# dan-lee-gh/monte-carlo-gp

Hardware: AMD Instinct MI355X
Metric: race-simulations/sec (20 drivers, 60 laps) (higher is better)
Workload: dtype f64

## Files before the change

monte_carlo_gp_amd/csrc/race_isa.hip.h:

```cpp
#ifndef MCGP_RACE_ISA_H
#define MCGP_RACE_ISA_H
#include <hip/hip_runtime.h>

namespace mcgp {

__device__ __forceinline__ void minmax_f64(double a, double b, double &lo, double &hi)
{
    asm("v_min_f64 %0, %1, %2" : "=v"(lo) : "v"(a), "v"(b));
    asm("v_max_f64 %0, %1, %2" : "=v"(hi) : "v"(a), "v"(b));
}

__device__ __forceinline__ double max_f64(double a, double b)
{
    double r;
    asm("v_max_f64 %0, %1, %2" : "=v"(r) : "v"(a), "v"(b));
    return r;
}

__device__ __forceinline__ double max_abs_f64(double a, double b)
{
    double r;
    asm("v_max_f64 %0, |%1|, %2" : "=v"(r) : "v"(a), "v"(b));
    return r;
}
// ... 627 lines not shown
__device__ __forceinline__ void lds_ld_u32x4(uint32_t addr, uint32_t &a, uint32_t &b, uint32_t &c, uint32_t &d)
{
    typedef uint32_t v4u __attribute__((ext_vector_type(4)));
    const v4u v = *reinterpret_cast<const MCGP_LDS v4u *>(addr);
    a = v.x; b = v.y; c = v.z; d = v.w;
}
__device__ __forceinline__ void lds_ld_f64_u32x2(uint32_t addr, double &d, uint32_t &u0, uint32_t &u1)
{
    typedef uint32_t v4u __attribute__((ext_vector_type(4)));
    const v4u v = *reinterpret_cast<const MCGP_LDS v4u *>(addr);
    d = __hiloint2double((int)v.y, (int)v.x);
    u0 = v.z;
    u1 = v.w;
}

__device__ __forceinline__ uint32_t cvt_u32_f64_sat(double x)
{
    uint32_t r;
    asm("v_cvt_u32_f64 %0, %1" : "=v"(r) : "v"(x));
    return r;
}
__device__ __forceinline__ double ceil_f64(double x) { return __builtin_ceil(x); }
__device__ __forceinline__ uint32_t min_u32(uint32_t a, uint32_t b) { return a < b ? a : b; }
__device__ __forceinline__ void sched_fence() { __builtin_amdgcn_sched_barrier(0); }
__device__ __forceinline__ void wave_sync()
{
    __builtin_amdgcn_fence(__ATOMIC_RELEASE, "wavefront");
    __builtin_amdgcn_wave_barrier();
    __builtin_amdgcn_fence(__ATOMIC_ACQUIRE, "wavefront");
}
// ... 49 lines not shown
```

monte_carlo_gp_amd/csrc/race_kernel_reg.hip.h:

```cpp
#pragma once
#include "race_common.hip.h"
#include "race_isa.hip.h"
#include "sort_networks.h"

#include <utility>

#ifndef MCGP_STAT
#define MCGP_STAT(what, value)
#endif
#ifndef MCGP_TRACE_PASS
#define MCGP_TRACE_PASS(sim, lap, pass, n_cand)
#endif
#ifndef MCGP_COOPERATIVE_EVENTS
#define MCGP_COOPERATIVE_EVENTS 1
#endif
#ifndef MCGP_GRID_EXACT
#define MCGP_GRID_EXACT 0
#endif
#ifndef MCGP_WIDE_EXACT
#define MCGP_WIDE_EXACT 0
#endif
#ifndef MCGP_WIDE_TIE_SHIFT
#define MCGP_WIDE_TIE_SHIFT 0
#endif

namespace mcgp {

constexpr uint32_t k3UsedMask = 7u;
constexpr uint32_t k3Drs = 1u << 3;
constexpr int k3IdShift = 4;
constexpr uint32_t k3IdMask = 31u << k3IdShift;
constexpr uint32_t k3Dnf = 1u << 9;
constexpr uint32_t k3SlotMask = k3IdMask | k3Dnf;
constexpr int k3CompShift = 10;
constexpr uint32_t k3CompMask = 7u << k3CompShift;
constexpr uint32_t k3Dirty = 1u << 13;
constexpr int k3AgeShift = 16;
constexpr uint32_t k3AgeMask = 0x7FFu << k3AgeShift;
constexpr int k3GposShift = 27;
__host__ __device__ constexpr uint32_t pk_driver16(uint32_t p) { return p & k3IdMask; }
__host__ __device__ constexpr uint32_t pk_slot16(uint32_t p) { return p & k3SlotMask; }
__host__ __device__ constexpr uint32_t pk_comp512(uint32_t p) { return (p & k3CompMask) >> (k3CompShift - 9); }
__host__ __device__ constexpr uint32_t pk_comp16(uint32_t p) { return (p >> (k3CompShift - 4)) & 0x70u; }
constexpr double kAgeFieldUnit = 1.0 / 65536.0;

constexpr size_t kLdsPerCu = 160 * 1024;
__host__ __device__ constexpr size_t align16(size_t x) { return (x + 15) / 16 * 16; }
constexpr int kWordRows = 8;
__host__ __device__ constexpr size_t per_thread_lds_bytes_reg(int n) { return (size_t)kWordRows * 4 + (size_t)n * 8; }
constexpr int kNumCompounds = 5;
__host__ __device__ constexpr size_t shared_lds_bytes_reg(int n)
{
    return (size_t)kNormalRows * 16 + (size_t)n * 16 + (size_t)(kMaxCars + n) * 16 +
           (size_t)((kNumCompounds - 1) * kMaxCars + n) * 16 + kCompStride * 16 + 64 + 128 + align16((size_t)n * n * 4) +
           align16((size_t)n * n * 8);
}
__host__ __device__ constexpr int reg_min_waves(int n) { return n <= 6 ? (n == 4 ? 4 : 6) : n <= 11 ? 4 : n <= 22 ? 3 : 2; }
__host__ __device__ constexpr bool reg_commit_by_selects(int n) { return n == 6 || (n >= 8 && n <= 10) || n == 24 || n == 25; }
__host__ __device__ constexpr bool reg_step_by_selects(int n) { return n == 3 || n == 11 || n == 12 || n == 25 || n == 26 || n == 29; }
__host__ __device__ constexpr bool reg_update_by_selects(int n)
{
    return n == 1 || n == 6 || (n >= 9 && n <= 11) || n == 22 || n == 28 || n == 29;
}
__host__ __device__ constexpr bool reg_threshold_by_selects(int n) { return n == 6 || n == 7 || (n >= 23 && n <= 25) || n >= 27; }
constexpr int kMaxBlockWaves = 16;
constexpr size_t kLdsReserve = 256;
__host__ __device__ constexpr int block_shape_rank(int w) { return (w % 4 == 0 ? 0 : 100) + (w <= 8 ? 2 * (8 - w) : w - 8); }
__host__ __device__ constexpr int reg_block_waves(int n)
{
    const int cap = 4 * reg_min_waves(n);
// ... 23 lines not shown
    return rows > kWideLdsRowsMax ? kWideLdsRowsMax : rows;
}
__host__ __device__ constexpr size_t wide_lds_bytes(int n, int waves)
{
    return wide_fixed_lds_bytes(n, waves) + (size_t)wide_lds_rows(n, waves) * kNorm53LdsStride;
}
__host__ __device__ constexpr size_t wide_chain_bytes(int n, int total_laps)
{
    return total_laps >= 2 ? (size_t)(total_laps - 1) * (size_t)((n + 3) & ~3) * 8 : 0;
}
__host__ __device__ constexpr size_t wide_launch_lds_bytes(int n, int waves, int total_laps)
{
    const size_t base = wide_lds_bytes(n, waves), chain = wide_chain_bytes(n, total_laps);
    return base + chain + kLdsReserve <= kLdsPerCu ? base + chain : base;
}
template <int N, int WAVES = reg_block_waves(N), bool WIDE = false>
struct RegGeo {
    static constexpr int kWaves = WAVES;
    static constexpr bool kWide = WIDE;
    static constexpr int B = 64 * kWaves;
    static constexpr uint32_t oDrvA = 0;
    static constexpr uint32_t oDrvB = oDrvA + N * 16;
    static constexpr uint32_t oIc = oDrvB + (kMaxCars + N) * 16;
    static constexpr uint32_t oComp = oIc + ((kNumCompounds - 1) * kMaxCars + N) * 16;
    static constexpr uint32_t oDrs = oComp + kCompStride * 16;
    static constexpr uint32_t oPit = oDrs + 16;
    static constexpr uint32_t oDrsB = oDrs + 32;
    static constexpr uint32_t oLut = oDrsB + 32;
    static constexpr uint32_t oNorm = oLut + 128;
    static constexpr uint32_t oHist = oNorm + (WIDE ? 0 : kNormalRows * 16);
    static_assert(WIDE || oNorm >= kNormalRowBias * 16, "the inverse-normal rows are addressed through a base 48 rows before the table");
    static constexpr uint32_t oGrid = oHist + (uint32_t)align16((size_t)N * N * 4);
    static constexpr uint32_t oW = oGrid + (uint32_t)align16((size_t)N * N * 8);
    static constexpr uint32_t oLast = oW + (uint32_t)kWordRows * B * 4;
    static constexpr uint32_t oNorm53 = oLast + (uint32_t)N * B * 8;
    static constexpr int kNorm53Rows = WIDE ? wide_lds_rows(N, WAVES) : 0;
    static constexpr int kNorm53First = kNormal53Rows - kNorm53Rows;
    static constexpr uint32_t kBytes = oNorm53 + (uint32_t)kNorm53Rows * (uint32_t)kNorm53LdsStride;
    static constexpr uint32_t oChain = kBytes;
    static constexpr uint32_t kChainStride = (uint32_t)((N + 3) & ~3) * 8u;
    __host__ __device__ static constexpr bool chain_fits(int total_laps)
    {
        return WIDE && total_laps >= 2 && kBytes + wide_chain_bytes(N, total_laps) + kLdsReserve <= kLdsPerCu;
    }
    static_assert(oW == shared_lds_bytes_reg(N) - (WIDE ? (size_t)kNormalRows * 16 : 0) && oLast % 8 == 0, "LDS map");
    static_assert(oW % 16 == 0 && oNorm53 % 16 == 0, "the event handler parks fields with 16-byte LDS accesses (ds_write_b128 / ds_read_b128); table rows are read 16 bytes at a time");
    static_assert(kBytes == (WIDE ? wide_lds_bytes(N, WAVES) : per_thread_lds_bytes_reg(N) * B + shared_lds_bytes_reg(N)), "LDS map");
    static_assert(kBytes + kLdsReserve <= kLdsPerCu, "block does not fit LDS");
// ... 1 lines not shown
};
constexpr int kWideMinLdsRows = 14 * 16;
__host__ __device__ constexpr int wide_block_waves(int n)
{
    if (n <= 22) {
        for (int w = 12; w > 8; --w)
            if (wide_fixed_lds_bytes(n, w) + kLdsReserve <= kLdsPerCu && wide_lds_rows(n, w) >= kWideMinLdsRows) return w;
    }
    int w = 8;
    while (w > 1 && wide_fixed_lds_bytes(n, w) + kLdsReserve > kLdsPerCu) --w;
    return w;
}
__host__ __device__ constexpr int wide_min_waves(int n) { return wide_block_waves(n) > 8 ? 3 : 2; }
template <int N>
using WideGeo = RegGeo<N, wide_block_waves(N), true>;

template <int N>
struct SortNetwork {
    int a[N * 8];
    int b[N * 8];
    int step[N * 8];
    int n;
    int ga[N * 8];
    int gn[N * 8];
    int n_groups;
    constexpr SortNetwork() : a{}, b{}, step{}, n(0), ga{}, gn{}, n_groups(0)
    {
        const SortNetworkTable *table = nullptr;
        for (const SortNetworkTable &t : kSortNetworks)
            if (t.n == N) table = &t;
// ... 188 lines not shown
}

template <int N>
__device__ __forceinline__ bool resort_after_overtakes(double (&cum)[N], uint32_t (&pk)[N])
{
    bubble_forward<N, 0>(cum, pk);
    bubble_backward<N, N - 2>(cum, pk);
    const bool strict = strictly_increasing<N>(cum);
    MCGP_STAT(14, !strict);
    if (__builtin_expect(!strict, 0)) {
        if (!in_order<N>(cum, pk)) transposition_sort<N>(cum, pk);
    }
    return strict;
}

template <int N, bool DISTINCT = false>
__device__ __forceinline__ void update_positions_reg(const double (&cum)[N], uint32_t (&pk)[N],
                                                     bool drs_allowed, double dirty_thr)
{
    bool first = true;
    double leader = 0.0, prev = 0.0;
#pragma unroll
    for (int i = 0; i < N; ++i) {
        const uint32_t p = pk[i];
        const bool act = !(p & k3Dnf);
        const double t = cum[i];
        leader = (act && first) ? t : leader;
        const double tbl = t - leader;
        const bool dirty = (DISTINCT ? !first : tbl > 0) && tbl < dirty_thr;
        const bool drs = !first && drs_allowed && (t - prev) < 1.0;
        pk[i] = (p & ~(k3Drs | k3Dirty)) | (dirty ? k3Dirty : 0u) | (drs ? k3Drs : 0u);
        prev = act ? t : prev;
        first = first && !act;
    }
}

__host__ __device__ constexpr int pit_regime(int remaining_laps)
{
    return remaining_laps > 30 ? 0 : remaining_laps > 20 ? 1 : remaining_laps > 15 ? 2 : 3;
}
__device__ __forceinline__ uint32_t pit_rule_word(int track, int regime, uint32_t used, uint32_t pop_sh, uint32_t pop_mh)
{
    const int remaining_laps = regime == 0 ? 31 : regime == 1 ? 21 : regime == 2 ? 16 : 0;
    uint32_t newc = stint_compound(track, remaining_laps);
    if (track == 0 && __popc(used) == 1 && ((used >> newc) & 1u)) {
        const uint32_t avail = 7u & ~used;
        const uint32_t popped = avail == 5u ? pop_sh : avail == 6u ? pop_mh : 0u;
        if (remaining_laps > 20) newc = (avail & 2u) ? 1u : popped;
        else newc = (avail & 1u) ? 0u : popped;
    }
    return (newc << k3CompShift) | ((used | (1u << newc)) & k3UsedMask);
}

constexpr double kRegTimeFloor = 8.0;
__host__ __device__ inline double reg_time_floor(const KParams &kp)
{
    const double z_max = kp.wide ? 8.5 : 6.5;
    double floor_ = __builtin_inf();
    double cdelta_min = __builtin_inf();
    for (int c = 0; c < 5; ++c) cdelta_min = kp.comp_delta[c] < cdelta_min ? kp.comp_delta[c] : cdelta_min;
    for (int d = 0; d < kp.n; ++d) {
        double eff_min = 0.0;
        for (int c = 0; c < 5; ++c) {
            const double e = kp.comp_deg[c] * kp.factor[d];
            eff_min = e < eff_min ? e : eff_min;
        }
// ... 42 lines not shown
            }
        }
    } else {
        float4 *t_norm = reinterpret_cast<float4 *>(smem + G::oNorm);
        for (uint32_t i = tid; i < (uint32_t)kNormalRows * 4; i += B)
            reinterpret_cast<uint32_t *>(t_norm)[i] = P->normal_bits[i];
    }
    for (uint32_t d = tid; d < (uint32_t)N; d += B) {
        double *a = reinterpret_cast<double *>(smem + G::oDrvA + d * 16);
        double *b = reinterpret_cast<double *>(smem + G::oDrvB + d * 16);
        const double qnan = __builtin_nan("");
        a[0] = P->variance[d];
        a[1] = P->base_pace[d];
        b[0] = P->base_pace[d] * 2147483648.0;
        b[1] = P->tire_deg[d] * 32768.0;
        b[2 * kMaxCars] = qnan;
        b[2 * kMaxCars + 1] = qnan;
    }
    if (tid < 2) {
        *reinterpret_cast<double *>(smem + G::oDrs + tid * k3Drs) = tid ? P->drs_delta : 0.0;
        *reinterpret_cast<double *>(smem + G::oDrsB + tid * k3Drs) = tid ? P->drs_delta * 2147483648.0 : 0.0;
        *reinterpret_cast<double *>(smem + G::oPit + tid * 8u) = tid ? P->pit_loss : 0.0;
    }
    for (uint32_t i = tid; i < (uint32_t)kNumCompounds * N; i += B) {
        const uint32_t c = i / N, d = i % N;
        unsigned char *r = smem + G::oIc + (c * kMaxCars + d) * 16;
        *reinterpret_cast<double *>(r) = (P->comp_deg[c] * P->factor[d]) * kAgeFieldUnit;
        *reinterpret_cast<uint32_t *>(r + 8) = (uint32_t)P->opt_laps[d * kCompStride + c] << 16;
        *reinterpret_cast<uint32_t *>(r + 12) = 0u;
    }
    for (uint32_t i = tid; i < 32u; i += B)
        *reinterpret_cast<uint32_t *>(smem + G::oLut + i * 4) =
            pit_rule_word(P->track, (int)(i >> 3), i & 7u, (uint32_t)P->pop_sh, (uint32_t)P->pop_mh);
    for (uint32_t c = tid; c < (uint32_t)kCompStride; c += B) {
        double *r = reinterpret_cast<double *>(smem + G::oComp + c * 16);
        r[0] = P->comp_delta[c];
        r[1] = 0.0;
    }
    for (uint32_t i = tid; i < (uint32_t)(N * N); i += B) {
        s_hist[i] = 0u;
        t_grid[(i % N) * N + (i / N)] = P->grid_probs[i];
    }
}

template <int N, class G = RegGeo<N>>
__device__ __forceinline__ void reg_flush_hist(unsigned char *smem, uint32_t tid, unsigned long long *__restrict__ hist)
{
    const uint32_t *s_hist = reinterpret_cast<const uint32_t *>(smem + G::oHist);
    for (uint32_t i = tid; i < (uint32_t)(N * N); i += G::B) {
        const uint32_t c = s_hist[i];
        if (c) atomicAdd(&hist[i], (unsigned long long)c);
    }
// ... 4 lines not shown
#if defined(__HIP_DEVICE_COMPILE__)
    return (uint32_t)__builtin_amdgcn_readfirstlane((int)x);
#else
    return x;
#endif
}
__device__ __forceinline__ uint32_t scalar_u32(uint32_t x)
{
    pin(x);
    return uniform_u32(x);
}
__device__ __forceinline__ double scalar_f64(double x)
{
    return __hiloint2double((int)scalar_u32((uint32_t)__double2hiint(x)), (int)scalar_u32((uint32_t)__double2loint(x)));
}
template <int N>
__device__ __forceinline__ void update_positions_distinct(const double (&cum)[N], uint32_t (&pk)[N], bool drs_allowed, double dirty_thr)
{
    if constexpr (reg_update_by_selects(N)) {
        update_positions_reg<N, true>(cum, pk, drs_allowed, dirty_thr);
    } else {
        const UpdLap c{scalar_f64(dirty_thr), lane_mask(drs_allowed)};
        uint64_t first = kAllLanes;
        double leader = 0.0, prev = 0.0;
        if constexpr (N >= 4) upd_commit4<k3Dnf, k3Dirty, k3Drs, true>(&cum[0], &pk[0], leader, prev, first, c);
        if constexpr (N == 3) upd_commit3<k3Dnf, k3Dirty, k3Drs, true>(&cum[0], &pk[0], leader, prev, first, c);
        if constexpr (N == 2) upd_commit2<k3Dnf, k3Dirty, k3Drs, true>(&cum[0], &pk[0], leader, prev, first, c);
        if constexpr (N == 1) upd_commit1<k3Dnf, k3Dirty, k3Drs, true>(&cum[0], &pk[0], leader, prev, first, c);
#pragma unroll
        for (int i0 = 4; i0 < N; i0 += 4) {
            const int K = N - i0 < 4 ? N - i0 : 4;
            if constexpr (N >= 8) if (K == 4) upd_commit4<k3Dnf, k3Dirty, k3Drs, false>(&cum[i0], &pk[i0], leader, prev, first, c);
            if constexpr (N > 4 && N % 4 == 3) if (K == 3) upd_commit3<k3Dnf, k3Dirty, k3Drs, false>(&cum[i0], &pk[i0], leader, prev, first, c);
            if constexpr (N > 4 && N % 4 == 2) if (K == 2) upd_commit2<k3Dnf, k3Dirty, k3Drs, false>(&cum[i0], &pk[i0], leader, prev, first, c);
            if constexpr (N > 4 && N % 4 == 1) if (K == 1) upd_commit1<k3Dnf, k3Dirty, k3Drs, false>(&cum[i0], &pk[i0], leader, prev, first, c);
        }
    }
}
template <int N, class G>
__device__ __forceinline__ uint32_t wide_pass_exact_body(const uint32_t (&pk)[N], double od31, uint32_t lap, uint32_t pass, uint32_t c0l,
                                                         uint32_t c1l, uint32_t k0l, uint32_t k1l, uint32_t tid)
{
    constexpr int B = G::B;
    const uint32_t tid4 = tid * 4u;
    auto w_row_ = [&](int r) -> uint32_t { return G::oW + (uint32_t)r * (B * 4) + tid4; };
    uint32_t hits53 = 0u;
    uint64_t thr64[N];
    uint32_t cand = 0u;
    {
        double pace_prev = 0.0;
#pragma unroll
        for (int i = 0; i < N; ++i) {
            const f64x2 bd = lds_ld_f64x2(G::oDrvB + pk_slot16(pk[i]));
            const double pace = bd.x + (double)(pk[i] & k3AgeMask) * bd.y;
            thr64[i] = 0ull;
            if (i > 0) {
                const double dl = (pace_prev - pace) + lds_ld<double>(G::oDrsB + (pk[i] & k3Drs));
                const bool c = dl > od31;
                double x = ceil_f64(dl * 0x1p21);
                x = x < 0x1p52 ? x : 0x1p52;
                const uint32_t xh = c ? cvt_u32_f64_sat(x * 0x1p-32) : 0u;
                const uint32_t xl = c ? cvt_u32_f64_sat(x - (double)xh * 0x1p32) : 0u;
                thr64[i] = ((uint64_t)xh << 32) | (uint64_t)xl;
                cand |= c ? (1u << i) : 0u;
            }
            pace_prev = pace;
        }
    }
// ... 54 lines not shown
        for (int j = 0; j < 4; ++j) at[j] += w[j] < S[j] ? span : 0u;
    }
#pragma unroll
    for (int j = 0; j < 4; ++j) survived[j] = at[j] / (uint32_t)sizeof(T);
}

template <int N, bool WIDE = false, class G = RegGeo<N>>
__device__ __forceinline__ void reg_simulate(const KParams *__restrict__ P, unsigned char *smem, uint32_t tid,
                                             uint32_t *__restrict__ ticket, uint64_t n_sims,
                                             uint64_t sim_offset, uint32_t seed_lo, uint32_t seed_hi,
                                             uint8_t *__restrict__ orders, const uint8_t *__restrict__ fixed_grid,
                                             uint32_t n_chunks, uint32_t *__restrict__ retire_ws_base, uint32_t ws_stride,
                                             uint32_t ws_first_lane, const double *__restrict__ norm53 = nullptr)
{
    constexpr int B = G::B;
    constexpr int kStepBatch = 4;
    constexpr bool kLean = WIDE && wide_min_waves(N) >= 3;
    constexpr int kPaceBatch = 5;
    static_assert(kStepBatch % 4 == 0, "a Philox block serves four consecutive places");
    const uint32_t tid4 = tid * 4u, tid8 = tid * 8u;
    const int L = P->total_laps;
    const int track = P->track;

    uint32_t *s_hist = reinterpret_cast<uint32_t *>(smem + G::oHist);

    auto w_row = [&](int r) -> uint32_t { return G::oW + (uint32_t)r * (B * 4) + tid4; };
    auto l_row = [&](int d) -> uint32_t { return G::oLast + (uint32_t)d * (B * 8) + tid8; };
    auto last_of = [&](uint32_t p) -> uint32_t { return ((p >> k3IdShift) & 31u) * (uint32_t)(B * 8) + tid8; };
    auto grid_byte = [&](int pos) -> uint32_t { return G::oW + (uint32_t)(pos >> 2) * (B * 4) + tid4 + (uint32_t)(pos & 3); };
    auto norm_row = [&](uint32_t off) -> float4 { return lds_ld_float4(G::oNorm - kNormalRowBias * 16u + off); };
// ... 14 lines not shown
        if (__builtin_expect(MCGP_ANY(G::kNorm53Rows == 0 || MCGP_WIDE_EXACT || hi < kRareHi), 0)) return normal53(w, x, norm53);
        double c[8];
        norm53_row(hi, c);
        return normal53_evaluate(w, c, t);
    };

    const double dirty_thr = P->dirty_thr;
    const float kNaN = __uint_as_float(0x7fc00000u);

    struct SlotIn {
        uint32_t pitw;
        double last, var, base, eff, cdelta, drs;
        uint32_t la;
        uint32_t fit;
    };
    auto load_slot = [&](uint32_t p, uint32_t lut_base) -> SlotIn {
        SlotIn r;
        r.fit = lds_ld<uint32_t>(((p & k3UsedMask) << 2) + lut_base);
        const uint32_t id16 = pk_driver16(p);
        r.la = id16 * (uint32_t)(B / 2) + tid8;
        r.last = lds_ld<double>(G::oLast + r.la);
        const uint32_t ic = id16 + pk_comp512(p);
        const f64x2 vb = lds_ld_f64x2(G::oDrvA + id16);
        r.var = vb.x;
        r.base = vb.y;
        uint32_t pad;
        lds_ld_f64_u32x2(G::oIc + ic, r.eff, r.pitw, pad);
        r.cdelta = lds_ld<double>(G::oComp + pk_comp16(p));
        r.drs = lds_ld<double>(G::oDrs + (p & k3Drs));
        return r;
    };

    for (uint32_t turn = 0u;; ++turn) {
        const uint32_t chunk = next_ticket(ticket, tid, turn, G::kWaves);
        if (chunk >= n_chunks) break;
        const uint64_t local = (uint64_t)chunk * 64ull + (uint64_t)(tid & 63u);
        const bool live = local < n_sims;
        if (!MCGP_ANY(live)) continue;
        const uint64_t sim = sim_offset + local;
        const uint32_t c0 = (uint32_t)sim, c1 = (uint32_t)(sim >> 32);

        double cum[N];
        uint32_t pk[N];

// ... 86 lines not shown
        if constexpr (WIDE) {
#pragma unroll 1
            for (int d = 0; d < N; ++d) {
                uint32_t w0, w1, w2, w3, x0, x1, x2, x3;
                philox4x32_10(c0, c1, 1u, kPurposeCar | (uint32_t)d, seed_lo, seed_hi, w0, w1, w2, w3);
                philox4x32_10(c0, c1, 1u, kPurposeCar | kCompanion | (uint32_t)d, seed_lo, seed_hi, x0, x1, x2, x3);
                const bool out = uniform53(w0, x0) < P->t53_dnf1[d];
                lds_st<double>(l_row(d), out ? __builtin_nan("") : normal53_one(w1, x1));
            }
#pragma unroll
            for (int i = 0; i < N; ++i) {
                const uint32_t p = pk[i];
                const double z = lds_ld<double>(G::oLast + last_of(p));
                const uint32_t id16 = pk_driver16(p);
                const f64x2 vb = lds_ld_f64x2(G::oDrvA + id16);
                const double eff = lds_ld<double>(G::oIc + id16 + pk_comp512(p));
                const double cdelta = lds_ld<double>(G::oComp + pk_comp16(p));
                if (z != z) {
                    pk[i] = (p & ~k3AgeMask) | k3Dnf | (1u << k3AgeShift);
                    cum[i] = -(double)(i + 1) * 0x1p-1000;
                } else {
                    const double tire = (double)(p & k3AgeMask) * eff;
                    const double fuel_effect = (110.0 - 110.0) * 0.03;
                    const double noise = 0.0 + vb.x * z;
                    cum[i] = vb.y + tire - fuel_effect + cdelta - 0.0 + noise;
                }
            }
#pragma unroll 1
            for (int d = 0; d < N; ++d) {
                uint32_t w0, w1, w2, w3, x0, x1, x2, x3;
                philox4x32_10(c0, c1, 1u, kPurposeCar | (uint32_t)d, seed_lo, seed_hi, w0, w1, w2, w3);
                philox4x32_10(c0, c1, 1u, kPurposeCar | kCompanion | (uint32_t)d, seed_lo, seed_hi, x0, x1, x2, x3);
// ... 17 lines not shown
            for (int d = 0; d < N; ++d) {
                uint32_t w0, w1, w2, w3;
                philox4x32_10(c0, c1, 1u, kPurposeCar | (uint32_t)d, seed_lo, seed_hi, w0, w1, w2, w3);
                const bool out = (uint64_t)w0 < P->t_dnf1[d];
                lds_st<float>(l_row(d), out ? kNaN : normal_from_u32_rows(w1, norm_row));
                lds_st<float>(l_row(d) + 4u, normal_from_u32_rows(w2, norm_row));
            }
#pragma unroll
            for (int i = 0; i < N; ++i) {
                const uint32_t p = pk[i];
                const uint32_t la = last_of(p);
                const float z = lds_ld<float>(G::oLast + la);
                const double zs = (double)lds_ld<float>(G::oLast + la + 4u);
                const uint32_t id16 = pk_driver16(p);
                const f64x2 vb = lds_ld_f64x2(G::oDrvA + id16);
                const double eff = lds_ld<double>(G::oIc + id16 + pk_comp512(p));
                const double cdelta = lds_ld<double>(G::oComp + pk_comp16(p));
                if (z != z) {
                    pk[i] = (p & ~k3AgeMask) | k3Dnf | (1u << k3AgeShift);
                    cum[i] = -(double)(i + 1) * 0x1p-1000;
                } else {
                    const double tire = (double)(p & k3AgeMask) * eff;
                    const double fuel_effect = (110.0 - 110.0) * 0.03;
                    const double noise = 0.0 + vb.x * (double)z;
                    const double base_lap = vb.y + tire - fuel_effect + cdelta - 0.0 + noise;
                    double pf = 0.5 + (double)(i + 1) * 0.1;
                    if (!(pf < 1.5)) pf = 1.5;
                    double sd = 0.0 + pf * zs;
                    if (i + 1 <= 3 && 1.0 < sd) sd = 1.0;
                    cum[i] = 0.0 + (base_lap - sd * 0.5);
                    pk[i] = p + (1u << k3AgeShift);
                }
            }
        }
#pragma unroll 1
        for (int d = 0; d < N; ++d) lds_st<double>(l_row(d), 0.0);
        network_sort<N>(cum, pk);
        update_positions_reg<N>(cum, pk, false, dirty_thr);

        constexpr uint32_t kNoKey = 0x7FFFu;
        auto retirements_after = [&](const uint32_t *ws, uint32_t after) -> uint32_t {
            const uint32_t n_out = ws[(size_t)N * ws_stride];
            uint32_t k1 = kNoKey, k2 = kNoKey, left = 0u;
#pragma unroll 1
            for (uint32_t k = 0; k < n_out; ++k) {
                const uint32_t e = ws[(size_t)k * ws_stride];
                if (e > after) {
                    ++left;
                    const uint32_t hi = e > k1 ? e : k1;
                    k1 = e < k1 ? e : k1;
                    k2 = hi < k2 ? hi : k2;
                }
            }
// ... 389 lines not shown
                    for (int j = 0; j < kStepBatch; ++j) {
                        const int i = i0 + j;
                        if (i >= N) continue;
                        const SlotIn &s = in[j];
                        const uint32_t p = pk[i];
                        const bool active = !(p & k3Dnf);
                        const bool dnf_hit = __double2hiint(s.last) < 0;
                        const bool run = active && !dnf_hit;
                        const double ahead_last = carry;
                        carry = active ? s.last : carry;
                        const uint32_t agef = p & k3AgeMask;
                        const double tire = (double)agef * s.eff;
                        const double drs_gain = s.drs;
                        const double noise = s.var * (double)z[j];
                        const double clean = s.base + tire - fuel_effect + s.cdelta - drs_gain + noise;
                        const uint32_t dirty_m = (uint32_t)((int32_t)(p << (31 - 13)) >> 31);
                        const double pen_if_dirty = __hiloint2double((int)((uint32_t)__double2hiint(dirty_pen_lap) & dirty_m),
                                                                     (int)((uint32_t)__double2loint(dirty_pen_lap) & dirty_m));
                        const double ahead_if_dirty = __hiloint2double((int)((uint32_t)__double2hiint(ahead_last) & dirty_m),
                                                                       (int)((uint32_t)__double2loint(ahead_last) & dirty_m));
                        const double lap_time = max_abs_f64(ahead_if_dirty, clean + pen_if_dirty);
                        const bool pit = run && pit_window && agef >= s.pitw;
                        const uint32_t p_pit = (p & ~(k3CompMask | k3UsedMask | k3AgeMask)) | s.fit;
                        uint32_t p_run = pit ? p_pit : p + (1u << k3AgeShift);
                        uint32_t p_ret = (p & ~k3AgeMask) | retire_word;
                        pin(p_run);
                        pin(p_ret);
                        const uint32_t p_act = dnf_hit ? p_ret : p_run;
                        pk[i] = active ? p_act : p;
                        const double lap_add = run ? lap_time : 0.0;
                        const double pit_add = lds_ld<double>(G::oPit + (pit ? 8u : 0u));
// ... 34 lines not shown
                        lds_st<uint32_t>(w_row(5), o1);
                        lds_st<uint32_t>(w_row(6), o2);
                        lds_st<uint32_t>(w_row(7), o3);
                    }
                    uint32_t row = tid4;
                    {
                        constexpr int H = kPaceBatch;
                            double pace_prev = 0.0;
#pragma unroll
                        for (int h = 0; h < N; h += H) {
                            sched_fence();
                            double pb[H], pd[H], pa[H];
#pragma unroll
                            for (int j = 0; j < H; ++j) {
                                if (h + j < N) {
                                    const uint32_t id16 = pk_slot16(pk[h + j]);
                                    const f64x2 bd = lds_ld_f64x2(G::oDrvB + id16);
                                    pb[j] = bd.x;
                                    pd[j] = bd.y;
                                    pa[j] = lds_ld<double>(G::oDrsB + (pk[h + j] & k3Drs));
                                }
                            }
#pragma unroll
                            for (int j = 0; j < H; ++j) {
                                const int i = h + j;
                                if (i < N) {
                                    const double pace = pb[j] + (double)(pk[i] & k3AgeMask) * pd[j];
                                    if (i > 0) {
                                        const double dl = (pace_prev - pace) + pa[j];
                                        if constexpr (reg_threshold_by_selects(N)) {
                                            uint32_t next;
// ... 80 lines not shown
                        any_succ |= hit;
                    }
                } else {
                    uint64_t hit_lanes = 0u;
                    overtake_commits<N, 1>(cum, ow, thr, hit_lanes);
                    any_succ = ovt_lane_hit(hit_lanes);
                }
                MCGP_STAT(4 + pass, any_succ);
                MCGP_STAT(8, n_attempts);
                MCGP_TRACE_PASS(local, lap, pass, (int)n_attempts);
                (void)n_attempts;
                if (!any_succ) break;
                distinct_times = resort_after_overtakes<N>(cum, pk);
            }
            if (!MCGP_ANY(!distinct_times))
                update_positions_distinct<N>(cum, pk, lap > 2 && lap > drs_disabled_until, dirty_thr);
            else
                update_positions_reg<N>(cum, pk, lap > 2 && lap > drs_disabled_until, dirty_thr);
        }

        uint32_t key[N];
        {
            uint32_t g = 0u;
#pragma unroll
            for (int i = 0; i < N; ++i) {
                if (i > 0) g += cum[i] != cum[i - 1] ? 1u : 0u;
                const uint32_t p = pk[i];
                const uint32_t id = (p >> k3IdShift) & 31u;
                const uint32_t lapf = (p >> k3AgeShift) & 0x7FFu;
                const uint32_t key_dnf = (1u << 26) | ((2047u - lapf) << 15) | ((31u - g) << 10) | ((p >> k3GposShift) << 5) | id;
                const uint32_t key_run = ((uint32_t)i << 5) | id;
                key[i] = (p & k3Dnf) ? key_dnf : key_run;
            }
// ... 51 lines not shown
    __syncthreads();
    reg_simulate<N, true, G>(P, smem, threadIdx.x, ticket, n_sims, sim_offset, seed_lo, seed_hi, orders, fixed_grid, n_chunks,
                             retire_ws, (uint32_t)(gridDim.x * G::B), (uint32_t)(blockIdx.x * G::B), norm53);
    __syncthreads();
    reg_flush_hist<N, G>(smem, threadIdx.x, hist);
}

struct BatchItem {
    uint64_t sim_offset, seed;
};
template <int N>
__device__ __forceinline__ void batch_problem(const KParams *__restrict__ P, unsigned char *smem, uint32_t *__restrict__ ticket,
                                              uint64_t n_sims, uint64_t sim_offset, uint64_t seed, uint32_t n_chunks,
                                              uint32_t *__restrict__ retire_ws, unsigned long long *__restrict__ hist)
{
    using G = RegGeo<N>;
    reg_load_tables<N>(P, smem, threadIdx.x);
    __syncthreads();
    reg_simulate<N>(P, smem, threadIdx.x, ticket, n_sims, sim_offset, (uint32_t)seed, (uint32_t)(seed >> 32),
                    nullptr, nullptr, n_chunks, retire_ws, (uint32_t)(gridDim.x * G::B), (uint32_t)(blockIdx.x * G::B));
    __syncthreads();
    reg_flush_hist<N>(smem, threadIdx.x, hist);
    __syncthreads();
}
template <int N>
__global__ void __launch_bounds__(RegGeo<N>::B, reg_min_waves(N))
race_kernel_reg_batch(const KParams *__restrict__ P, const BatchItem *__restrict__ items, uint32_t n_problems,
                      uint64_t n_sims, unsigned long long *__restrict__ hist, uint32_t n_chunks,
                      uint32_t *__restrict__ tickets, uint32_t *__restrict__ retire_ws, uint32_t param_stride)
{
    using G = RegGeo<N>;
    extern __shared__ __align__(16) unsigned char smem[];
    if ((int)blockDim.x != G::B || lds_base_of(smem) != 0u) __builtin_trap();
    uint32_t p = (uint32_t)(((uint64_t)blockIdx.x * n_problems) / gridDim.x);
    uint32_t visited = 0u;
    for (;;) {
        if (threadIdx.x < 64u) {
            uint32_t found = 0xFFFFFFFFu, seen = visited;
            while (seen < n_problems) {
                const uint32_t k = seen + threadIdx.x;
                uint32_t q = p + (k - visited);
                if (q >= n_problems) q -= n_problems;
                const uint32_t lane = first_lane_with(k < n_problems && peek_ticket(&tickets[q]) < n_chunks);
                if (lane < 64u) {
                    found = seen + lane;
                    break;
// ... 22 lines not shown
```

Before: 164.3 million.

## Relay LDS tables and pk word bits to pair compound/DRS loads

Computes a per-N LDS table layout at compile time that moves the DNF and dirty flag bits in the packed driver word and relocates the tables. The DNF bit then doubles as a byte offset to a NaN copy of the pace table, and the compound index maps directly to a table offset. For N up to 30 it interleaves compound delta and DRS delta into pair rows, so one ds_read2_b64-style load fetches both values and the per-slot address arithmetic shrinks. Some N keep the old layout via an exception list, and the batch kernel gets its own geometry; the risk is extra complexity and different LDS bank and alignment behaviour.

```diff
diff --git a/monte_carlo_gp_amd/csrc/race_isa.hip.h b/monte_carlo_gp_amd/csrc/race_isa.hip.h
--- a/monte_carlo_gp_amd/csrc/race_isa.hip.h
+++ b/monte_carlo_gp_amd/csrc/race_isa.hip.h
@@ -665,6 +665,14 @@
     u1 = v.w;
 }
 
+template <uint32_t BASE>
+__device__ __forceinline__ void lds_ld2_f64(uint32_t addr, double &a, double &b)
+{
+    static_assert(BASE % 8 == 0 && BASE / 8 + 2 <= 255, "ds_read2_b64 offsets");
+    a = lds_ld<double>(BASE + addr);
+    b = lds_ld<double>(BASE + 16u + addr);
+}
+
 __device__ __forceinline__ uint32_t cvt_u32_f64_sat(double x)
 {
     uint32_t r;
diff --git a/monte_carlo_gp_amd/csrc/race_kernel_reg.hip.h b/monte_carlo_gp_amd/csrc/race_kernel_reg.hip.h
--- a/monte_carlo_gp_amd/csrc/race_kernel_reg.hip.h
+++ b/monte_carlo_gp_amd/csrc/race_kernel_reg.hip.h
@@ -30,18 +30,10 @@
 constexpr uint32_t k3Drs = 1u << 3;
 constexpr int k3IdShift = 4;
 constexpr uint32_t k3IdMask = 31u << k3IdShift;
-constexpr uint32_t k3Dnf = 1u << 9;
-constexpr uint32_t k3SlotMask = k3IdMask | k3Dnf;
-constexpr int k3CompShift = 10;
-constexpr uint32_t k3CompMask = 7u << k3CompShift;
-constexpr uint32_t k3Dirty = 1u << 13;
 constexpr int k3AgeShift = 16;
 constexpr uint32_t k3AgeMask = 0x7FFu << k3AgeShift;
 constexpr int k3GposShift = 27;
 __host__ __device__ constexpr uint32_t pk_driver16(uint32_t p) { return p & k3IdMask; }
-__host__ __device__ constexpr uint32_t pk_slot16(uint32_t p) { return p & k3SlotMask; }
-__host__ __device__ constexpr uint32_t pk_comp512(uint32_t p) { return (p & k3CompMask) >> (k3CompShift - 9); }
-__host__ __device__ constexpr uint32_t pk_comp16(uint32_t p) { return (p >> (k3CompShift - 4)) & 0x70u; }
 constexpr double kAgeFieldUnit = 1.0 / 65536.0;
 
 constexpr size_t kLdsPerCu = 160 * 1024;
@@ -54,6 +46,93 @@
     return (size_t)kNormalRows * 16 + (size_t)n * 16 + (size_t)(kMaxCars + n) * 16 +
            (size_t)((kNumCompounds - 1) * kMaxCars + n) * 16 + kCompStride * 16 + 64 + 128 + align16((size_t)n * n * 4) +
            align16((size_t)n * n * 8);
+}
+struct RegTables {
+    bool relaid;
+    bool pair;
+    int comp_shift;
+    uint32_t dnf, dirty;
+    uint32_t oDrvA, oDrvB, oIc, oComp, oDrs, oLut, oNorm, oHist, oGrid, end;
+};
+enum RegKind { kRegDefault = 0, kRegBatch = 1, kRegWide = 2 };
+__host__ __device__ constexpr bool reg_pk_earlier_layout(int n, int kind)
+{
+    return kind == kRegBatch  ? n == 5 || n == 6 || n == 13 || n == 16 || (n >= 20 && n <= 22)
+           : kind == kRegWide ? n == 9 || n == 10 || n == 21
+                              : n == 6 || n == 9 || n == 21;
+}
+__host__ __device__ constexpr RegTables reg_tables(int n, int kind)
+{
+    const bool wide = kind == kRegWide;
+    const uint32_t un = (uint32_t)n;
+    const uint32_t total = (uint32_t)shared_lds_bytes_reg(n) - (wide ? (uint32_t)kNormalRows * 16u : 0u);
+    const uint32_t sz_norm = wide ? 0u : (uint32_t)kNormalRows * 16u, sz_hist = (uint32_t)align16((size_t)n * n * 4),
+                   sz_grid = (uint32_t)align16((size_t)n * n * 8);
+    RegTables t{};
+    t.relaid = false;
+    t.pair = false;
+    t.comp_shift = 10;
+    t.dnf = 1u << 9;
+    t.dirty = 1u << 13;
+    t.oDrvA = 0;
+    t.oDrvB = t.oDrvA + un * 16u;
+    t.oIc = t.oDrvB + ((uint32_t)kMaxCars + un) * 16u;
+    t.oComp = t.oIc + ((uint32_t)(kNumCompounds - 1) * kMaxCars + un) * 16u;
+    t.oDrs = t.oComp + (uint32_t)kCompStride * 16u;
+    t.oLut = t.oDrs + 64u;
+    t.oNorm = t.oLut + 128u;
+    t.oHist = t.oNorm + sz_norm;
+    t.oGrid = t.oHist + sz_hist;
+    t.end = t.oGrid + sz_grid;
+    if (reg_pk_earlier_layout(n, kind)) return t;
+
+    const bool pair = n <= 30;
+    const uint32_t sz_ic = ((uint32_t)(kNumCompounds - 1) * kMaxCars + un) * 16u + (pair ? 32u : 0u), sz_pace = un * 16u;
+    constexpr int kItems = 7;
+    const uint32_t sz[kItems] = {sz_norm, un * 16u, 64u, 128u, pair ? 0u : (uint32_t)kCompStride * 16u, sz_hist, sz_grid};
+    uint32_t sum_all = 0;
+    for (int k = 0; k < kItems; ++k) sum_all += sz[k];
+    uint32_t best_waste = ~0u, best_set = 0, best_dist = 0;
+    bool best_ic_first = true;
+    for (uint32_t dist = 8192u; dist >= 4096u; dist >>= 1)
+        for (int head = 0; head < 2; ++head) {
+            const bool ic_first = head == 0;
+            const uint32_t fixed = sz_pace + (ic_first ? 0u : sz_ic);
+            if (fixed > dist) continue;
+            for (uint32_t set = 0; set < (1u << kItems); ++set) {
+                uint32_t in = 0;
+                for (int k = 0; k < kItems; ++k) in += (set >> k) & 1u ? sz[k] : 0u;
+                if (fixed + in > dist) continue;
+                const uint32_t waste = dist - fixed - in;
+                const uint32_t end = (ic_first ? sz_ic : 0u) + dist + sz_pace + (sum_all - in);
+                if (end <= total && waste < best_waste) { best_waste = waste; best_set = set; best_dist = dist; best_ic_first = ic_first; }
+            }
+        }
+    if (best_dist == 0) return t;
+
+    t.relaid = true;
+    t.pair = pair;
+    t.comp_shift = 9;
+    t.dnf = best_dist;
+    t.dirty = best_dist == 8192u ? 4096u : 8192u;
+    t.oIc = best_ic_first ? 0u : sz_pace;
+    t.oDrvB = best_ic_first ? sz_ic : 0u;
+    uint32_t in_span = sz_ic + sz_pace, behind = t.oDrvB + best_dist + sz_pace;
+    uint32_t at[kItems] = {};
+    for (int k = 0; k < kItems; ++k) {
+        uint32_t &cursor = (best_set >> k) & 1u ? in_span : behind;
+        at[k] = cursor;
+        cursor += sz[k];
+    }
+    t.oNorm = at[0];
+    t.oDrvA = at[1];
+    t.oDrs = at[2];
+    t.oLut = at[3];
+    t.oComp = at[4];
+    t.oHist = at[5];
+    t.oGrid = at[6];
+    t.end = behind;
+    return t;
 }
 __host__ __device__ constexpr int reg_min_waves(int n) { return n <= 6 ? (n == 4 ? 4 : 6) : n <= 11 ? 4 : n <= 22 ? 3 : 2; }
 __host__ __device__ constexpr bool reg_commit_by_selects(int n) { return n == 6 || (n >= 8 && n <= 10) || n == 24 || n == 25; }
@@ -107,24 +186,38 @@
     const size_t base = wide_lds_bytes(n, waves), chain = wide_chain_bytes(n, total_laps);
     return base + chain + kLdsReserve <= kLdsPerCu ? base + chain : base;
 }
-template <int N, int WAVES = reg_block_waves(N), bool WIDE = false>
+template <int N, int WAVES = reg_block_waves(N), bool WIDE = false, int KIND = WIDE ? kRegWide : kRegDefault>
 struct RegGeo {
     static constexpr int kWaves = WAVES;
     static constexpr bool kWide = WIDE;
     static constexpr int B = 64 * kWaves;
-    static constexpr uint32_t oDrvA = 0;
-    static constexpr uint32_t oDrvB = oDrvA + N * 16;
-    static constexpr uint32_t oIc = oDrvB + (kMaxCars + N) * 16;
-    static constexpr uint32_t oComp = oIc + ((kNumCompounds - 1) * kMaxCars + N) * 16;
-    static constexpr uint32_t oDrs = oComp + kCompStride * 16;
+    static_assert(WIDE == (KIND == kRegWide), "RegKind");
+    static constexpr RegTables T = reg_tables(N, KIND);
+    static constexpr uint32_t oDrvA = T.oDrvA;
+    static constexpr uint32_t oDrvB = T.oDrvB;
+    static constexpr uint32_t oIc = T.oIc;
+    static constexpr uint32_t oPair = oIc + N * 16;
+    static constexpr uint32_t oComp = T.oComp;
+    static constexpr uint32_t oDrs = T.oDrs;
     static constexpr uint32_t oPit = oDrs + 16;
     static constexpr uint32_t oDrsB = oDrs + 32;
-    static constexpr uint32_t oLut = oDrsB + 32;
-    static constexpr uint32_t oNorm = oLut + 128;
-    static constexpr uint32_t oHist = oNorm + (WIDE ? 0 : kNormalRows * 16);
+    static constexpr uint32_t oLut = T.oLut;
+    static constexpr uint32_t oNorm = T.oNorm;
+    static constexpr uint32_t oHist = T.oHist;
+    static constexpr bool kRelaid = T.relaid, kPair = T.pair;
+    static constexpr uint32_t kDnf = T.dnf, kDirty = T.dirty;
+    static constexpr int kCompShift = T.comp_shift;
+    static constexpr uint32_t kCompMask = 7u << kCompShift;
+    static constexpr uint32_t kSlotMask = k3IdMask | kDnf;
+    static constexpr uint32_t kIcMask = k3IdMask | kCompMask;
+    static constexpr uint32_t kPairMask = kCompMask | k3Drs;
+    static_assert(T.end <= shared_lds_bytes_reg(N) - (WIDE ? (size_t)kNormalRows * 16 : 0), "the table map ends within the bytes the launch has always had");
+    static_assert(!kRelaid || (kCompShift == 9 && (kDnf == 4096u || kDnf == 8192u) && (kDnf | kDirty) == 0x3000u), "pk word");
+    static_assert(!kPair || (kRelaid && N <= 30 && oPair % 8 == 0 && oPair / 8 + 2 <= 255), "pair rows: in oIc's padding, base within the ds_read2_b64 offsets");
+    static_assert((kSlotMask & ~k3IdMask) == kDnf && kDnf % 16 == 0, "the NaN copy of the overtake pace lies kDnf bytes after the live table");
     static_assert(WIDE || oNorm >= kNormalRowBias * 16, "the inverse-normal rows are addressed through a base 48 rows before the table");
-    static constexpr uint32_t oGrid = oHist + (uint32_t)align16((size_t)N * N * 4);
-    static constexpr uint32_t oW = oGrid + (uint32_t)align16((size_t)N * N * 8);
+    static constexpr uint32_t oGrid = T.oGrid;
+    static constexpr uint32_t oW = (uint32_t)shared_lds_bytes_reg(N) - (WIDE ? (uint32_t)kNormalRows * 16u : 0u);
     static constexpr uint32_t oLast = oW + (uint32_t)kWordRows * B * 4;
     static constexpr uint32_t oNorm53 = oLast + (uint32_t)N * B * 8;
     static constexpr int kNorm53Rows = WIDE ? wide_lds_rows(N, WAVES) : 0;
@@ -156,6 +249,8 @@
 __host__ __device__ constexpr int wide_min_waves(int n) { return wide_block_waves(n) > 8 ? 3 : 2; }
 template <int N>
 using WideGeo = RegGeo<N, wide_block_waves(N), true>;
+template <int N>
+using BatchGeo = RegGeo<N, reg_block_waves(N), false, kRegBatch>;
 
 template <int N>
 struct SortNetwork {
@@ -374,10 +469,11 @@
     return strict;
 }
 
-template <int N, bool DISTINCT = false>
+template <int N, class G, bool DISTINCT = false>
 __device__ __forceinline__ void update_positions_reg(const double (&cum)[N], uint32_t (&pk)[N],
                                                      bool drs_allowed, double dirty_thr)
 {
+    constexpr uint32_t k3Dnf = G::kDnf, k3Dirty = G::kDirty;
     bool first = true;
     double leader = 0.0, prev = 0.0;
 #pragma unroll
@@ -399,7 +495,7 @@
 {
     return remaining_laps > 30 ? 0 : remaining_laps > 20 ? 1 : remaining_laps > 15 ? 2 : 3;
 }
-__device__ __forceinline__ uint32_t pit_rule_word(int track, int regime, uint32_t used, uint32_t pop_sh, uint32_t pop_mh)
+__device__ __forceinline__ uint32_t pit_rule_word(int track, int regime, uint32_t used, uint32_t pop_sh, uint32_t pop_mh, int comp_shift)
 {
     const int remaining_laps = regime == 0 ? 31 : regime == 1 ? 21 : regime == 2 ? 16 : 0;
     uint32_t newc = stint_compound(track, remaining_laps);
@@ -409,7 +505,7 @@
         if (remaining_laps > 20) newc = (avail & 2u) ? 1u : popped;
         else newc = (avail & 1u) ? 0u : popped;
     }
-    return (newc << k3CompShift) | ((used | (1u << newc)) & k3UsedMask);
+    return (newc << comp_shift) | ((used | (1u << newc)) & k3UsedMask);
 }
 
 constexpr double kRegTimeFloor = 8.0;
@@ -482,11 +578,11 @@
         a[1] = P->base_pace[d];
         b[0] = P->base_pace[d] * 2147483648.0;
         b[1] = P->tire_deg[d] * 32768.0;
-        b[2 * kMaxCars] = qnan;
-        b[2 * kMaxCars + 1] = qnan;
+        b[G::kDnf / 8] = qnan;
+        b[G::kDnf / 8 + 1] = qnan;
     }
     if (tid < 2) {
-        *reinterpret_cast<double *>(smem + G::oDrs + tid * k3Drs) = tid ? P->drs_delta : 0.0;
+        if constexpr (!G::kPair) *reinterpret_cast<double *>(smem + G::oDrs + tid * k3Drs) = tid ? P->drs_delta : 0.0;
         *reinterpret_cast<double *>(smem + G::oDrsB + tid * k3Drs) = tid ? P->drs_delta * 2147483648.0 : 0.0;
         *reinterpret_cast<double *>(smem + G::oPit + tid * 8u) = tid ? P->pit_loss : 0.0;
     }
@@ -499,11 +595,21 @@
     }
     for (uint32_t i = tid; i < 32u; i += B)
         *reinterpret_cast<uint32_t *>(smem + G::oLut + i * 4) =
-            pit_rule_word(P->track, (int)(i >> 3), i & 7u, (uint32_t)P->pop_sh, (uint32_t)P->pop_mh);
-    for (uint32_t c = tid; c < (uint32_t)kCompStride; c += B) {
-        double *r = reinterpret_cast<double *>(smem + G::oComp + c * 16);
-        r[0] = P->comp_delta[c];
-        r[1] = 0.0;
+            pit_rule_word(P->track, (int)(i >> 3), i & 7u, (uint32_t)P->pop_sh, (uint32_t)P->pop_mh, G::kCompShift);
+    if constexpr (G::kPair) {
+        for (uint32_t c = tid; c < (uint32_t)kNumCompounds; c += B) {
+            double *r = reinterpret_cast<double *>(smem + G::oPair + c * (kMaxCars * 16u));
+            r[0] = P->comp_delta[c];
+            r[1] = P->comp_delta[c];
+            r[2] = 0.0;
+            r[3] = P->drs_delta;
+        }
+    } else {
+        for (uint32_t c = tid; c < (uint32_t)kCompStride; c += B) {
+            double *r = reinterpret_cast<double *>(smem + G::oComp + c * 16);
+            r[0] = P->comp_delta[c];
+            r[1] = 0.0;
+        }
     }
     for (uint32_t i = tid; i < (uint32_t)(N * N); i += B) {
         s_hist[i] = 0u;
@@ -538,11 +644,12 @@
 {
     return __hiloint2double((int)scalar_u32((uint32_t)__double2hiint(x)), (int)scalar_u32((uint32_t)__double2loint(x)));
 }
-template <int N>
+template <int N, class G>
 __device__ __forceinline__ void update_positions_distinct(const double (&cum)[N], uint32_t (&pk)[N], bool drs_allowed, double dirty_thr)
 {
+    constexpr uint32_t k3Dnf = G::kDnf, k3Dirty = G::kDirty;
     if constexpr (reg_update_by_selects(N)) {
-        update_positions_reg<N, true>(cum, pk, drs_allowed, dirty_thr);
+        update_positions_reg<N, G, true>(cum, pk, drs_allowed, dirty_thr);
     } else {
         const UpdLap c{scalar_f64(dirty_thr), lane_mask(drs_allowed)};
         uint64_t first = kAllLanes;
@@ -566,6 +673,7 @@
                                                          uint32_t c1l, uint32_t k0l, uint32_t k1l, uint32_t tid)
 {
     constexpr int B = G::B;
+    constexpr uint32_t k3SlotMask = G::kSlotMask;
     const uint32_t tid4 = tid * 4u;
     auto w_row_ = [&](int r) -> uint32_t { return G::oW + (uint32_t)r * (B * 4) + tid4; };
     uint32_t hits53 = 0u;
@@ -575,7 +683,7 @@
         double pace_prev = 0.0;
 #pragma unroll
         for (int i = 0; i < N; ++i) {
-            const f64x2 bd = lds_ld_f64x2(G::oDrvB + pk_slot16(pk[i]));
+            const f64x2 bd = lds_ld_f64x2(G::oDrvB + (pk[i] & k3SlotMask));
             const double pace = bd.x + (double)(pk[i] & k3AgeMask) * bd.y;
             thr64[i] = 0ull;
             if (i > 0) {
@@ -660,6 +768,8 @@
                                              uint32_t ws_first_lane, const double *__restrict__ norm53 = nullptr)
 {
     constexpr int B = G::B;
+    constexpr uint32_t k3Dnf = G::kDnf, k3Dirty = G::kDirty, k3CompMask = G::kCompMask, k3SlotMask = G::kSlotMask;
+    constexpr int k3CompShift = G::kCompShift;
     constexpr int kStepBatch = 4;
     constexpr bool kLean = WIDE && wide_min_waves(N) >= 3;
     constexpr int kPaceBatch = 5;
@@ -704,20 +814,32 @@
         uint32_t la;
         uint32_t fit;
     };
+    auto ic_of = [&](uint32_t p) -> uint32_t {
+        if constexpr (G::kRelaid) return p & G::kIcMask;
+        else return pk_driver16(p) + ((p & k3CompMask) >> (k3CompShift - 9));
+    };
+    auto cdelta_at = [&](uint32_t p) -> uint32_t {
+        if constexpr (G::kPair) return G::oPair + (p & k3CompMask);
+        else return G::oComp + ((p >> (k3CompShift - 4)) & 0x70u);
+    };
     auto load_slot = [&](uint32_t p, uint32_t lut_base) -> SlotIn {
         SlotIn r;
         r.fit = lds_ld<uint32_t>(((p & k3UsedMask) << 2) + lut_base);
         const uint32_t id16 = pk_driver16(p);
         r.la = id16 * (uint32_t)(B / 2) + tid8;
         r.last = lds_ld<double>(G::oLast + r.la);
-        const uint32_t ic = id16 + pk_comp512(p);
+        const uint32_t ic = ic_of(p);
         const f64x2 vb = lds_ld_f64x2(G::oDrvA + id16);
         r.var = vb.x;
         r.base = vb.y;
         uint32_t pad;
         lds_ld_f64_u32x2(G::oIc + ic, r.eff, r.pitw, pad);
-        r.cdelta = lds_ld<double>(G::oComp + pk_comp16(p));
-        r.drs = lds_ld<double>(G::oDrs + (p & k3Drs));
+        if constexpr (G::kPair) {
+            lds_ld2_f64<G::oPair>(p & G::kPairMask, r.cdelta, r.drs);
+        } else {
+            r.cdelta = lds_ld<double>(cdelta_at(p));
+            r.drs = lds_ld<double>(G::oDrs + (p & k3Drs));
+        }
         return r;
     };
 
@@ -834,8 +956,8 @@
                 const double z = lds_ld<double>(G::oLast + last_of(p));
                 const uint32_t id16 = pk_driver16(p);
                 const f64x2 vb = lds_ld_f64x2(G::oDrvA + id16);
-                const double eff = lds_ld<double>(G::oIc + id16 + pk_comp512(p));
-                const double cdelta = lds_ld<double>(G::oComp + pk_comp16(p));
+                const double eff = lds_ld<double>(G::oIc + ic_of(p));
+                const double cdelta = lds_ld<double>(cdelta_at(p));
                 if (z != z) {
                     pk[i] = (p & ~k3AgeMask) | k3Dnf | (1u << k3AgeShift);
                     cum[i] = -(double)(i + 1) * 0x1p-1000;
@@ -883,8 +1005,8 @@
                 const double zs = (double)lds_ld<float>(G::oLast + la + 4u);
                 const uint32_t id16 = pk_driver16(p);
                 const f64x2 vb = lds_ld_f64x2(G::oDrvA + id16);
-                const double eff = lds_ld<double>(G::oIc + id16 + pk_comp512(p));
-                const double cdelta = lds_ld<double>(G::oComp + pk_comp16(p));
+                const double eff = lds_ld<double>(G::oIc + ic_of(p));
+                const double cdelta = lds_ld<double>(cdelta_at(p));
                 if (z != z) {
                     pk[i] = (p & ~k3AgeMask) | k3Dnf | (1u << k3AgeShift);
                     cum[i] = -(double)(i + 1) * 0x1p-1000;
@@ -905,7 +1027,7 @@
 #pragma unroll 1
         for (int d = 0; d < N; ++d) lds_st<double>(l_row(d), 0.0);
         network_sort<N>(cum, pk);
-        update_positions_reg<N>(cum, pk, false, dirty_thr);
+        update_positions_reg<N, G>(cum, pk, false, dirty_thr);
 
         constexpr uint32_t kNoKey = 0x7FFFu;
         auto retirements_after = [&](const uint32_t *ws, uint32_t after) -> uint32_t {
@@ -1325,7 +1447,7 @@
                         const double drs_gain = s.drs;
                         const double noise = s.var * (double)z[j];
                         const double clean = s.base + tire - fuel_effect + s.cdelta - drs_gain + noise;
-                        const uint32_t dirty_m = (uint32_t)((int32_t)(p << (31 - 13)) >> 31);
+                        const uint32_t dirty_m = (uint32_t)((int32_t)(p << (k3Dirty == 8192u ? 31 - 13 : 31 - 12)) >> 31);
                         const double pen_if_dirty = __hiloint2double((int)((uint32_t)__double2hiint(dirty_pen_lap) & dirty_m),
                                                                      (int)((uint32_t)__double2loint(dirty_pen_lap) & dirty_m));
                         const double ahead_if_dirty = __hiloint2double((int)((uint32_t)__double2hiint(ahead_last) & dirty_m),
@@ -1390,7 +1512,7 @@
 #pragma unroll
                             for (int j = 0; j < H; ++j) {
                                 if (h + j < N) {
-                                    const uint32_t id16 = pk_slot16(pk[h + j]);
+                                    const uint32_t id16 = pk[h + j] & k3SlotMask;
                                     const f64x2 bd = lds_ld_f64x2(G::oDrvB + id16);
                                     pb[j] = bd.x;
                                     pd[j] = bd.y;
@@ -1501,9 +1623,9 @@
                 distinct_times = resort_after_overtakes<N>(cum, pk);
             }
             if (!MCGP_ANY(!distinct_times))
-                update_positions_distinct<N>(cum, pk, lap > 2 && lap > drs_disabled_until, dirty_thr);
+                update_positions_distinct<N, G>(cum, pk, lap > 2 && lap > drs_disabled_until, dirty_thr);
             else
-                update_positions_reg<N>(cum, pk, lap > 2 && lap > drs_disabled_until, dirty_thr);
+                update_positions_reg<N, G>(cum, pk, lap > 2 && lap > drs_disabled_until, dirty_thr);
         }
 
         uint32_t key[N];
@@ -1585,22 +1707,22 @@
                                               uint64_t n_sims, uint64_t sim_offset, uint64_t seed, uint32_t n_chunks,
                                               uint32_t *__restrict__ retire_ws, unsigned long long *__restrict__ hist)
 {
-    using G = RegGeo<N>;
-    reg_load_tables<N>(P, smem, threadIdx.x);
+    using G = BatchGeo<N>;
+    reg_load_tables<N, G>(P, smem, threadIdx.x);
     __syncthreads();
-    reg_simulate<N>(P, smem, threadIdx.x, ticket, n_sims, sim_offset, (uint32_t)seed, (uint32_t)(seed >> 32),
-                    nullptr, nullptr, n_chunks, retire_ws, (uint32_t)(gridDim.x * G::B), (uint32_t)(blockIdx.x * G::B));
+    reg_simulate<N, false, G>(P, smem, threadIdx.x, ticket, n_sims, sim_offset, (uint32_t)seed, (uint32_t)(seed >> 32),
+                              nullptr, nullptr, n_chunks, retire_ws, (uint32_t)(gridDim.x * G::B), (uint32_t)(blockIdx.x * G::B));
     __syncthreads();
-    reg_flush_hist<N>(smem, threadIdx.x, hist);
+    reg_flush_hist<N, G>(smem, threadIdx.x, hist);
     __syncthreads();
 }
 template <int N>
-__global__ void __launch_bounds__(RegGeo<N>::B, reg_min_waves(N))
+__global__ void __launch_bounds__(BatchGeo<N>::B, reg_min_waves(N))
 race_kernel_reg_batch(const KParams *__restrict__ P, const BatchItem *__restrict__ items, uint32_t n_problems,
                       uint64_t n_sims, unsigned long long *__restrict__ hist, uint32_t n_chunks,
                       uint32_t *__restrict__ tickets, uint32_t *__restrict__ retire_ws, uint32_t param_stride)
 {
-    using G = RegGeo<N>;
+    using G = BatchGeo<N>;
     extern __shared__ __align__(16) unsigned char smem[];
     if ((int)blockDim.x != G::B || lds_base_of(smem) != 0u) __builtin_trap();
     uint32_t p = (uint32_t)(((uint64_t)blockIdx.x * n_problems) / gridDim.x);
```

After: 167.2 million (median of 6 runs). +1.8%, better.
